# see--/speech_recognition

Measured on AMD Instinct MI355X. Metric: 1s 16kHz clips/sec training throughput, higher is better.
Workload: dtype f32; 1 GPU; configs[1]: 12-class conv_1d_time_sliced_with_attention, batch 1024/GPU synthetic 16000-sample fp32 clips, sampler+augment+STFT/mel(80,60)+raw fwd/bwd+RMSprop; global_batch=1024, parallelism=dp1, clip_bank=65536

## Files before the change

### include/kws_hip.h

```cpp
#ifndef KWS_HIP_H_
#define KWS_HIP_H_

#include <stdint.h>

#ifdef __cplusplus
extern "C" {
#endif
#if defined(__GNUC__) || defined(__clang__)
#pragma GCC visibility push(default)
#endif

#define KWS_OK 0
#define KWS_E_INVALID (-1)
#define KWS_E_HIP (-2)
#define KWS_E_WORKSPACE (-3)

#define KWS_ABI_VERSION 5

int kws_abi_version(void);
const char* kws_last_error(void);
int kws_device_name(char* buf, int cap);

int kws_stream_create(int cls, void** stream);
int kws_stream_destroy(void* stream);
// ... 186 lines not shown
                       void* stream);
int kws_conv1d_dgrad_f32(const float* dY, const float* W, float* dX, int accumulate, const kws_conv1d_t* d, void* stream);
int64_t kws_conv1d_wgrad_workspace_floats(const kws_conv1d_t* d);
int kws_conv1d_wgrad_f32(const float* X, const float* bn, const float* dY, float* dW, float* workspace, const kws_conv1d_t* d,
                         void* stream);

int kws_avgpool3_same_fwd_f32(const float* x, const float* bn, float* z, int B, int L, int C, void* stream);
int kws_avgpool3_same_bwd_f32(const float* dz, float* dx, int accumulate, int B, int L, int C, void* stream);

#define KWS_ACT_RELU6 0
#define KWS_ACT_RELU 1
typedef struct {
  int B, H, W, Hout, Wout;
  int kh, kw;
  int sh, sw;
  int dh, dw;
  int pad_t, pad_l;
  int Cin, F;
  int act;
} kws_conv2d_t;
int kws_conv2d_stats_rows(const kws_conv2d_t* d);
int kws_conv2d_fwd_f32(const float* X, const float* bn, const float* Wt, float* Y, float* stats_part, const kws_conv2d_t* d,
                       void* stream);
int kws_conv2d_dgrad_f32(const float* dY, const float* Wt, float* dX, const kws_conv2d_t* d, void* stream);
int64_t kws_conv2d_wgrad_workspace_floats(const kws_conv2d_t* d);
int kws_conv2d_wgrad_f32(const float* X, const float* bn, const float* dY, float* dWt, float* workspace, const kws_conv2d_t* d,
                         void* stream);

int kws_pool2x2_fwd_f32(const float* y, const float* bn, float* z, int B, int H, int W, int C, int act, void* stream);
int kws_pool2x2_bwd_part_rows(int B, int H, int W, int C);
int64_t kws_pool2x2_bwd_part_floats(int B, int H, int W, int C);
int kws_pool2x2_bwd_f32(const float* dz, const float* y, const float* bn, float* g, float* part, int B, int H, int W, int C, int act,
                        void* stream);

typedef struct {
  int B, L, Lout;
  int ksize, hop, pad_l;
  int taps, stride;
  int N;
  int64_t x_batch_stride;
} kws_frame_conv_t;
int kws_frame_conv_stats_rows(const kws_frame_conv_t* d);
int kws_frame_conv_fwd_f32(const float* x, const float* W, float* y, float* stats_part, const kws_frame_conv_t* d, void* stream);
int64_t kws_frame_conv_wgrad_workspace_floats(const kws_frame_conv_t* d);
int kws_frame_conv_wgrad_f32(const float* x, const float* G, float* dW, float* workspace, const kws_frame_conv_t* d, void* stream);

typedef struct {
  int B, L, Lout;
  int stride;
  int nbanks, N;
  int ksize[8], pad_l[8];
  int64_t w_off[8];
  int64_t x_batch_stride;
} kws_fbank_conv_t;
int     kws_fbank_conv_fwd_f32(const float* x, const float* W, float* y, const kws_fbank_conv_t* d, void* stream);
int64_t kws_fbank_conv_wgrad_workspace_floats(const kws_fbank_conv_t* d);
int     kws_fbank_conv_wgrad_f32(const float* x, const float* G, float* dW, float* workspace, const kws_fbank_conv_t* d, void* stream);

int kws_gap_drop_fwd_f32(const float* y, const float* bn, float* feat, float* fd, int B, int T, int C, float keep_prob, uint64_t seed,
                         uint32_t step, uint32_t layer_id, int64_t row_offset, void* stream);
int kws_gap_drop_bwd_part_rows(int B, int T, int C);
int kws_gap_drop_bwd_f32(const float* dfd, const float* y, const float* bn, float* g, float* part, int B, int T, int C, float keep_prob,
                         uint64_t seed, uint32_t step, uint32_t layer_id, int64_t row_offset, void* stream);

#define KWS_REDUCE_SLICES 32
int kws_bn_stats_finalize(const float* stats_part, int n_tiles, int64_t count, int C,
                          const float* gamma, const float* beta, float eps, float momentum,
                          float* moving_mean, float* moving_var, float* bn, float* scratch,
                          void* stream);
int kws_bn_infer_prepare(const float* gamma, const float* beta, const float* moving_mean,
                         const float* moving_var, float eps, int C, float* bn, void* stream);
int kws_bn_relu6_apply(const float* y, const float* bn, float* out, int64_t rows, int C, int relu6,
                       void* stream);

int kws_dwconv_fwd_f32(const float* y, const float* bn, const float* w, float* z, int B, int L_in,
                       int L_out, int C, int stride, int pad_l, void* stream);
int64_t kws_dwconv_bwd_part_floats(int B, int L_in, int C);
int kws_dwconv_bwd_f32(const float* dz, const float* y, const float* bn, const float* w, float* g,
                       float* part, int B, int L_in, int L_out, int C, int stride, int pad_l,
                       void* stream);
int kws_dwconv_bwd_bn_f32(const float* dz, const float* y, const float* bn, const float* w,
                          const float* coef, float* dy, float* part, int pass, int B, int L_in,
                          int L_out, int C, int stride, int pad_l, void* stream);
int kws_dw_bwd_finalize(const float* part, int n_parts, int64_t count, int C, float* dw,
                        float* dgamma, float* dbeta, float* coef, float* scratch, void* stream);
int kws_bn_bwd_apply(float* g, const float* y, const float* bn, const float* gamma,
                     const float* coef, int64_t rows, int C, void* stream);

int kws_dwconvk_fwd_f32(const float* y, const float* bn, const float* w, float* z, int B, int L_in, int L_out, int C,
                        int k, int stride, int pad_l, void* stream);
int kws_dwconvk_bwd_part_rows(int B, int L_in, int C, int k, int stride);
int64_t kws_dwconvk_bwd_part_floats(int B, int L_in, int C, int k, int stride);
int kws_dwconvk_bwd_f32(const float* dz, const float* y, const float* bn, const float* w, float* g, float* part, int B,
                        int L_in, int L_out, int C, int k, int stride, int pad_l, void* stream);
int kws_dwconvk_bwd_finalize(const float* part, int n_parts, int64_t count, int C, int k, float* dw, float* dgamma,
                             float* dbeta, float* coef, void* stream);
int kws_dwconvk_pw1_stats_rows(int64_t M);
int kws_dwconvk_pw1_fwd_f32(const float* z, const float* p, float* y, int64_t M, int N, float* stats_part, void* stream);
int64_t kws_dwconvk_pw1_bwd_workspace_floats(int64_t M, int N);
int kws_dwconvk_pw1_bwd_f32(const float* dy, const float* z, const float* p, float* dz, float* dp, int64_t M, int N,
                            float* workspace, void* stream);

int kws_stem_stats_rows(int B, int L);
int kws_stem_fwd_f32(const float* x, const float* w, const float* p, float* y, int B, int L, int C, int N, float* stats_part,
                     void* stream);
int64_t kws_stem_bwd_workspace_floats(int B, int L, int C, int N);
int kws_stem_bwd_f32(const float* dy, const float* x, const float* w, const float* p, float* dw, float* dp, int B, int L, int C,
                     int N, float* workspace, void* stream);

int64_t kws_gru_save_floats(int B, int T, int H);
int64_t kws_gru_workspace_floats(int B, int T, int I, int H, int backward);
int kws_gru_masks(float* mx, float* mh, int B, int I, int H, float keep_prob, uint64_t seed, uint32_t step, int64_t row_offset,
                  void* stream);
int kws_gru_seq_fwd_f32(const float* a, int64_t dir_stride, int64_t gate_stride, int row_stride, const float* U0, const float* U1,
                        const float* bias0, const float* bias1, const float* mh, float* out, float* save, int B, int T, int H,
                        void* stream);
int kws_gru_seq_bwd_f32(const float* dout, const float* UT, const float* mh, const float* save, float* da, float* lop, int B, int T,
                        int H, void* stream);
int kws_gru_fwd_f32(const float* x, const float* W0, const float* U0, const float* bias0, const float* W1, const float* U1,
                    const float* bias1, const float* mx, const float* mh, float* out, float* save, float* workspace, int B, int T,
                    int I, int H, void* stream);
int kws_gru_bwd_f32(const float* dout, const float* x, const float* W0, const float* U0, const float* W1, const float* U1,
                    const float* mx, const float* mh, const float* save, float* dx, float* dW0, float* dU0, float* dbias0, float* dW1,
                    float* dU1, float* dbias1, float* workspace, int B, int T, int I, int H, void* stream);

int64_t kws_attn_gate_fwd_floats(int B, int T, int C, int k);
int64_t kws_attn_gate_bwd_floats(int B, int T, int C, int k);
int kws_attn_gate_fwd_f32(const float* x, const float* wa, const float* Wa, const float* gamma, const float* beta, float* mm,
                          float* mv, float* u, float* table, float* att, float* y, float* workspace, int B, int T, int C, int k,
                          int training, void* stream);
int kws_attn_gate_bwd_f32(const float* dy, const float* x, const float* u, const float* att, const float* table, const float* wa,
                          const float* Wa, const float* gamma, float* dx, float* dwa, float* dWa, float* dgamma, float* dbeta,
                          float* workspace, int B, int T, int C, int k, int training, void* stream);

int kws_rmsprop_step(float* p, const float* grad, float* acc, const float* l2, int64_t n, float lr,
                     float rho, float eps, float grad_scale, void* stream);
int kws_sgd_momentum_step(float* p, const float* grad, float* vel, const float* l2, int64_t n,
                          float lr, float momentum, float grad_scale, void* stream);
int kws_adam_step(float* p, const float* grad, float* m, float* v, const float* l2, int64_t n, float lr_t,
                  float beta1, float beta2, float eps, float grad_scale, void* stream);
int kws_l2_loss(const float* p, const float* l2, int64_t n, float* out, void* stream);

#define KWS_NET_TS_ATTENTION 1
#define KWS_NET_LOG_MFCC 2
#define KWS_NET_STEFFE 3
#define KWS_NET_RESIDUAL 4
#define KWS_NET_MFCC_AND_RAW 5
#define KWS_NET_CONV_1D_FAST 6
#define KWS_NET_CONV_1D_SPEC 7
#define KWS_NET_CONV_1D_TIME_STACKED 8
#define KWS_NET_CONV_1D_HEAVY 9
#define KWS_NET_CONV_1D_GRU 10
#define KWS_NET_CONV_1D_MULTI_TIME_SLICED 11
#define KWS_NET_CONV_1D_SIMPLE 12
#define KWS_NET_XCEPTION_ATTENTION 13
#define KWS_NET_INCEPTION_D1 14
#define KWS_NET_CONV_2D_MOBILE 15
#define KWS_NET_CONV_2D_FAST 16
#define KWS_NET_CONV_1D_TIME_SLICED 17
#define KWS_NET_CONV_1D_LEARNED_SPEC 18
#define KWS_NET_CONV_1D_TOP_DOWN 19
typedef struct kws_net kws_net_t;
typedef struct {
  int kind;
  int num_classes;
  int filter_mult;
// ... 50 lines not shown
```

### speech_recognition_amd/_lib.py

```python
import ctypes
import os

_HERE = os.path.dirname(os.path.abspath(__file__))
LIB_PATH = os.environ.get("KWS_LIB_PATH") or os.path.join(_HERE, "libkws_hip.so")

ABI_VERSION = 5

KWS_NET_TS_ATTENTION = 1
KWS_NET_LOG_MFCC = 2
KWS_NET_STEFFE = 3
KWS_NET_RESIDUAL = 4
KWS_NET_MFCC_AND_RAW = 5
KWS_NET_CONV_1D_FAST = 6
KWS_NET_CONV_1D_SPEC = 7
KWS_NET_CONV_1D_TIME_STACKED = 8
KWS_NET_CONV_1D_HEAVY = 9
KWS_NET_CONV_1D_GRU = 10
KWS_NET_CONV_1D_MULTI_TIME_SLICED = 11
KWS_NET_CONV_1D_SIMPLE = 12
KWS_NET_XCEPTION_ATTENTION = 13
KWS_NET_INCEPTION_D1 = 14
KWS_NET_CONV_2D_MOBILE = 15
KWS_NET_CONV_2D_FAST = 16
KWS_NET_CONV_1D_TIME_SLICED = 17
# ... 145 lines not shown
    "kws_gemm_tn_f16x2_f32": (_I, [_P, _P, _P, _I64, _I, _I, _P, _P, _P, _P]),
    "kws_gemm_gather_f32": (_I, [_P, ctypes.POINTER(GatherDesc), _P, _P, _I, _I, _P, _P]),
    "kws_gemm_tn_workspace_floats": (_I64, [_I64, _I, _I]),
    "kws_gemm_tn_f32": (_I, [_P, _P, _P, _I64, _I, _I, _P, _P]),
    "kws_gemm_tn_gather_f32": (_I, [_P, ctypes.POINTER(GatherDesc), _P, _P, _I, _I, _P, _P]),
    "kws_gconv_stats_rows": (_I, [ctypes.POINTER(GconvDesc)]),
    "kws_gconv_fwd_f32": (_I, [_P, _P, _I, _P, _P, _P, ctypes.POINTER(GconvDesc), _P]),
    "kws_gconv_dgrad_f32": (_I, [_P, _P, _P, ctypes.POINTER(GconvDesc), _P]),
    "kws_gconv_wgrad_workspace_floats": (_I64, [ctypes.POINTER(GconvDesc)]),
    "kws_gconv_wgrad_f32": (_I, [_P, _P, _I, _P, _P, _P, ctypes.POINTER(GconvDesc), _P]),
    "kws_gdwconv_fwd_f32": (_I, [_P, _P, _P, _P, ctypes.POINTER(GdwconvDesc), _P]),
    "kws_gdwconv_bwd_part_rows": (_I, [ctypes.POINTER(GdwconvDesc)]),
    "kws_gdwconv_bwd_workspace_floats": (_I64, [ctypes.POINTER(GdwconvDesc)]),
    "kws_gdwconv_bwd_f32": (_I, [_P, _P, _P, _P, _P, _P, _P, _P, ctypes.POINTER(GdwconvDesc), _P]),
    "kws_pool3s2_out_len": (_I, [_I]),
    "kws_pool3s2_fwd_f32": (_I, [_P, _P, _P, _I, _I, _I, _P]),
    "kws_pool3s2_bwd_part_rows": (_I, [_I, _I, _I]),
    "kws_pool3s2_bwd_part_floats": (_I64, [_I, _I, _I]),
    "kws_pool3s2_bwd_f32": (_I, [_P, _P, _P, _P, _P, _I, _I, _I, _P]),
    "kws_pool3s2_same_out_len": (_I, [_I]),
    "kws_pool3s2_same_fwd_f32": (_I, [_P, _P, _P, _I, _I, _I, _P]),
    "kws_pool3s2_same_bwd_part_rows": (_I, [_I, _I, _I]),
    "kws_pool3s2_same_bwd_part_floats": (_I64, [_I, _I, _I]),
    "kws_pool3s2_same_bwd_f32": (_I, [_P, _P, _P, _P, _P, _I, _I, _I, _P]),
    "kws_conv1d_stats_rows": (_I, [ctypes.POINTER(Conv1dDesc)]),
    "kws_conv1d_fwd_f32": (_I, [_P, _P, _P, _P, _P, ctypes.POINTER(Conv1dDesc), _P]),
    "kws_conv1d_dgrad_f32": (_I, [_P, _P, _P, _I, ctypes.POINTER(Conv1dDesc), _P]),
    "kws_conv1d_wgrad_workspace_floats": (_I64, [ctypes.POINTER(Conv1dDesc)]),
    "kws_conv1d_wgrad_f32": (_I, [_P, _P, _P, _P, _P, ctypes.POINTER(Conv1dDesc), _P]),
    "kws_conv2d_stats_rows": (_I, [ctypes.POINTER(Conv2dDesc)]),
    "kws_conv2d_fwd_f32": (_I, [_P, _P, _P, _P, _P, ctypes.POINTER(Conv2dDesc), _P]),
    "kws_conv2d_dgrad_f32": (_I, [_P, _P, _P, ctypes.POINTER(Conv2dDesc), _P]),
    "kws_conv2d_wgrad_workspace_floats": (_I64, [ctypes.POINTER(Conv2dDesc)]),
    "kws_conv2d_wgrad_f32": (_I, [_P, _P, _P, _P, _P, ctypes.POINTER(Conv2dDesc), _P]),
    "kws_pool2x2_fwd_f32": (_I, [_P, _P, _P, _I, _I, _I, _I, _I, _P]),
    "kws_pool2x2_bwd_part_rows": (_I, [_I, _I, _I, _I]),
    "kws_pool2x2_bwd_part_floats": (_I64, [_I, _I, _I, _I]),
    "kws_pool2x2_bwd_f32": (_I, [_P, _P, _P, _P, _P, _I, _I, _I, _I, _I, _P]),
    "kws_frame_conv_stats_rows": (_I, [ctypes.POINTER(FrameConvDesc)]),
    "kws_frame_conv_fwd_f32": (_I, [_P, _P, _P, _P, ctypes.POINTER(FrameConvDesc), _P]),
    "kws_frame_conv_wgrad_workspace_floats": (_I64, [ctypes.POINTER(FrameConvDesc)]),
    "kws_frame_conv_wgrad_f32": (_I, [_P, _P, _P, _P, ctypes.POINTER(FrameConvDesc), _P]),
    "kws_fbank_conv_fwd_f32": (_I, [_P, _P, _P, ctypes.POINTER(FbankConvDesc), _P]),
    "kws_fbank_conv_wgrad_workspace_floats": (_I64, [ctypes.POINTER(FbankConvDesc)]),
    "kws_fbank_conv_wgrad_f32": (_I, [_P, _P, _P, _P, ctypes.POINTER(FbankConvDesc), _P]),
    "kws_gap_drop_fwd_f32": (_I, [_P, _P, _P, _P, _I, _I, _I, _F, ctypes.c_uint64, ctypes.c_uint32, ctypes.c_uint32, _I64, _P]),
    "kws_gap_drop_bwd_part_rows": (_I, [_I, _I, _I]),
    "kws_gap_drop_bwd_f32": (_I, [_P, _P, _P, _P, _P, _I, _I, _I, _F, ctypes.c_uint64, ctypes.c_uint32, ctypes.c_uint32, _I64,
                                  _P]),
    "kws_avgpool3_same_fwd_f32": (_I, [_P, _P, _P, _I, _I, _I, _P]),
    "kws_avgpool3_same_bwd_f32": (_I, [_P, _P, _I, _I, _I, _I, _P]),
    "kws_stem_stats_rows": (_I, [_I, _I]),
    "kws_stem_fwd_f32": (_I, [_P, _P, _P, _P, _I, _I, _I, _I, _P, _P]),
    "kws_stem_bwd_workspace_floats": (_I64, [_I, _I, _I, _I]),
    "kws_stem_bwd_f32": (_I, [_P, _P, _P, _P, _P, _P, _I, _I, _I, _I, _P, _P]),
    "kws_dwconvk_fwd_f32": (_I, [_P, _P, _P, _P, _I, _I, _I, _I, _I, _I, _I, _P]),
    "kws_dwconvk_bwd_part_rows": (_I, [_I, _I, _I, _I, _I]),
    "kws_dwconvk_bwd_part_floats": (_I64, [_I, _I, _I, _I, _I]),
    "kws_dwconvk_bwd_f32": (_I, [_P, _P, _P, _P, _P, _P, _I, _I, _I, _I, _I, _I, _I, _P]),
    "kws_dwconvk_bwd_finalize": (_I, [_P, _I, _I64, _I, _I, _P, _P, _P, _P, _P]),
    "kws_dwconvk_pw1_stats_rows": (_I, [_I64]),
    "kws_dwconvk_pw1_fwd_f32": (_I, [_P, _P, _P, _I64, _I, _P, _P]),
    "kws_dwconvk_pw1_bwd_workspace_floats": (_I64, [_I64, _I]),
    "kws_dwconvk_pw1_bwd_f32": (_I, [_P, _P, _P, _P, _P, _I64, _I, _P, _P]),
    "kws_gru_save_floats": (_I64, [_I, _I, _I]),
    "kws_gru_workspace_floats": (_I64, [_I, _I, _I, _I, _I]),
    "kws_gru_masks": (_I, [_P, _P, _I, _I, _I, _F, ctypes.c_uint64, ctypes.c_uint32, _I64, _P]),
    "kws_gru_seq_fwd_f32": (_I, [_P, _I64, _I64, _I, _P, _P, _P, _P, _P, _P, _P, _I, _I, _I, _P]),
    "kws_gru_seq_bwd_f32": (_I, [_P, _P, _P, _P, _P, _P, _I, _I, _I, _P]),
    "kws_gru_fwd_f32": (_I, [_P] * 12 + [_I, _I, _I, _I, _P]),
    "kws_gru_bwd_f32": (_I, [_P] * 17 + [_I, _I, _I, _I, _P]),
    "kws_attn_gate_fwd_floats": (_I64, [_I, _I, _I, _I]),
    "kws_attn_gate_bwd_floats": (_I64, [_I, _I, _I, _I]),
    "kws_attn_gate_fwd_f32": (_I, [_P] * 12 + [_I, _I, _I, _I, _I, _P]),
    "kws_attn_gate_bwd_f32": (_I, [_P] * 14 + [_I, _I, _I, _I, _I, _P]),
    "kws_transpose_f32": (_I, [_P, _P, _I, _I, _P]),
    "kws_bn_stats_finalize": (_I, [_P, _I, _I64, _I, _P, _P, _F, _F, _P, _P, _P, _P, _P]),
    "kws_bn_infer_prepare": (_I, [_P, _P, _P, _P, _F, _I, _P, _P]),
    "kws_bn_relu6_apply": (_I, [_P, _P, _P, _I64, _I, _I, _P]),
    "kws_dwconv_fwd_f32": (_I, [_P, _P, _P, _P, _I, _I, _I, _I, _I, _I, _P]),
    "kws_dwconv_bwd_part_floats": (_I64, [_I, _I, _I]),
    "kws_dwconv_bwd_f32": (_I, [_P, _P, _P, _P, _P, _P, _I, _I, _I, _I, _I, _I, _P]),
    "kws_dwconv_bwd_bn_f32": (_I, [_P, _P, _P, _P, _P, _P, _P, _I, _I, _I, _I, _I, _I, _I, _P]),
    "kws_dw_bwd_finalize": (_I, [_P, _I, _I64, _I, _P, _P, _P, _P, _P, _P]),
    "kws_bn_bwd_apply": (_I, [_P, _P, _P, _P, _P, _I64, _I, _P]),
    "kws_rmsprop_step": (_I, [_P, _P, _P, _P, _I64, _F, _F, _F, _F, _P]),
    "kws_sgd_momentum_step": (_I, [_P, _P, _P, _P, _I64, _F, _F, _F, _P]),
    "kws_adam_step": (_I, [_P, _P, _P, _P, _P, _I64, _F, _F, _F, _F, _F, _P]),
    "kws_l2_loss": (_I, [_P, _P, _I64, _P, _P]),
    "kws_net_create": (_I, [ctypes.POINTER(NetConfig), ctypes.POINTER(_P)]),
    "kws_net_destroy": (_I, [_P]),
    "kws_net_num_params": (_I64, [_P]),
    "kws_net_num_state": (_I64, [_P]),
    "kws_net_num_tensors": (_I, [_P]),
    "kws_net_tensor_info": (_I, [_P, _I, ctypes.POINTER(TensorInfo)]),
    "kws_net_workspace_bytes": (_I64, [_P, _I, _I]),
    "kws_net_debug_view": (_I, [_P, _I, _I, _I, _I, ctypes.POINTER(_I64), ctypes.POINTER(_I64)]),
    "kws_net_predict": (_I, [_P, _P, _P, _P, _I, _P, _P, _I64, _P]),
    "kws_net_train_fwd_bwd": (_I, [_P, _P, _P, _P, _P, _I, _P, _P, _P, ctypes.c_uint64, ctypes.c_uint32,
                                   _I64, _I, _P, _I64, _P]),
    "kws_net_num_blocks": (_I, [_P]),
    "kws_net_grad_ready_offset": (_I64, [_P, _I]),
    "kws_net_train_fwd_bwd_part": (_I, [_P, _P, _P, _P, _P, _I, _P, _P, _P, ctypes.c_uint64, ctypes.c_uint32,
                                        _I64, _I, _P, _I64, _I, _I, _P]),
}

_lib = None


def load():
    global _lib
    if _lib is not None:
        return _lib
    if not os.path.exists(LIB_PATH):
        raise KwsError("libkws_hip.so not found at %s - build it with "
                       "`python -c 'import __graft_entry__ as g; g.build()'` "
                       "(there is no CPU fallback)" % LIB_PATH)
    lib = ctypes.CDLL(LIB_PATH)
    lib.kws_abi_version.restype = _I
    if lib.kws_abi_version() != ABI_VERSION:
        raise KwsError("%s has ABI version %d, this package expects %d - rebuild it (__graft_entry__.build())" %
                       (LIB_PATH, lib.kws_abi_version(), ABI_VERSION))
    for name, (res, args) in SIGNATURES.items():
        fn = getattr(lib, name)
        fn.restype = res
        fn.argtypes = args
    _lib = lib
    return lib


def check(rc, what=""):
    if rc != 0:
        msg = load().kws_last_error()
        raise KwsError("%s failed (%d): %s" % (what or "libkws_hip call", rc,
                                               msg.decode() if msg else "?"))


def ptr(t):
    if t is None:
        return None
    return ctypes.c_void_p(t.data_ptr())


def stream_ptr(stream=None):
    import torch
    s = stream if stream is not None else torch.cuda.current_stream()
    return ctypes.c_void_p(s.cuda_stream)


class OwnedStream(object):

    def __init__(self, device, cls):
        import torch
        self.device = device
        with torch.cuda.device(device):
            h = ctypes.c_void_p()
            check(load().kws_stream_create(int(cls), ctypes.byref(h)), "kws_stream_create")
            self.handle = h.value
            self.stream = torch.cuda.ExternalStream(h.value, device=device)

    def close(self):
        h, self.handle = self.handle, None
        if h and _lib is not None:
            try:
                import torch
                with torch.cuda.device(self.device):
# ... 55 lines not shown
```

### speech_recognition_amd/csrc/dw_bwd_body.h

```cpp
#pragma once
#include "internal.h"

namespace kws_dw {

#ifndef KWS_DW_NT
#define KWS_DW_NT 1
#endif
typedef float dw_v4f __attribute__((ext_vector_type(4)));
__device__ __forceinline__ float4 ld4_stream(const float* p) {
  if (KWS_DW_NT & 2) {
    const dw_v4f v = __builtin_nontemporal_load(reinterpret_cast<const dw_v4f*>(p));
    return make_float4(v.x, v.y, v.z, v.w);
  }
  return *reinterpret_cast<const float4*>(p);
}
__device__ __forceinline__ void st4_stream(float* p, float4 o) {
  if (KWS_DW_NT & 1) {
    dw_v4f v = {o.x, o.y, o.z, o.w};
    __builtin_nontemporal_store(v, reinterpret_cast<dw_v4f*>(p));
    return;
  }
  *reinterpret_cast<float4*>(p) = o;
}

#ifndef KWS_DW_TT
#define KWS_DW_TT 8
#endif
constexpr int TT = KWS_DW_TT;

__device__ __forceinline__ float4 f4_fma(float4 a, float4 b, float4 c) {
  return make_float4(fmaf(a.x, b.x, c.x), fmaf(a.y, b.y, c.y), fmaf(a.z, b.z, c.z), fmaf(a.w, b.w, c.w));
}
__device__ __forceinline__ float4 f4_mul(float4 a, float4 b) {
  return make_float4(a.x * b.x, a.y * b.y, a.z * b.z, a.w * b.w);
}
__device__ __forceinline__ float4 f4_zero() { return make_float4(0.f, 0.f, 0.f, 0.f); }

#ifndef DW_BWD_THREADS
#define DW_BWD_THREADS 512
#endif
#ifndef DW_BWD_HT
#define DW_BWD_HT 8
#endif
#ifndef DW_BWD2_THREADS
#define DW_BWD2_THREADS 512
#endif
#ifndef DW_BWD_PARTS
#define DW_BWD_PARTS 256
#endif

struct BwdArgs {
  const float* dz; const float* y; const float* bn; const float* w; const float* coef;
  float* g; float* part;
  int B, Lin, Lout, C, pad_l, nchunks, R, Cb;
  unsigned* amax;
  int add_stride = 0, add_len = 0;
};
constexpr int bwd_smem_floats(int mode, int threads) { return mode == 2 ? 4 : 5 * threads * 4; }

template <int S, bool HAS_BN, int MODE, bool GUARD, bool ADDS = false>
__device__ __forceinline__ void bwd_body(const BwdArgs& p, float* const red, const int bid, const int nblk, const int by) {
  const float* __restrict__ dz = p.dz;
  const float* __restrict__ y = p.y;
  const float* __restrict__ bn = p.bn;
  const float* __restrict__ w = p.w;
  const float* __restrict__ coef = p.coef;
  float* __restrict__ g = p.g;
  float* __restrict__ part = p.part;
  const int B = p.B, Lin = p.Lin, Lout = p.Lout, C = p.C, pad_l = p.pad_l, nchunks = p.nchunks, R = p.R, Cb = p.Cb;
  constexpr int RSTRIDE = (MODE == 2 ? 4 : DW_BWD_THREADS * 4);
  float gmax = 0.f;
  const int C4 = Cb >> 2;
  const int tid = threadIdx.x;
  const bool live = !GUARD || tid < R * C4;
  const int r = live ? tid / C4 : 0, c4 = live ? tid - r * C4 : 0;
  const int c = by * Cb + c4 * 4;
  float4 sg = f4_zero(), sgx = f4_zero(), sw0 = f4_zero(), sw1 = f4_zero(), sw2 = f4_zero();
  float4 sc = f4_zero(), sh = f4_zero(), mean = f4_zero(), rstd = f4_zero();
  if (HAS_BN) {
    sc = *reinterpret_cast<const float4*>(bn + c);
    sh = *reinterpret_cast<const float4*>(bn + C + c);
    mean = *reinterpret_cast<const float4*>(bn + 2 * C + c);
    rstd = *reinterpret_cast<const float4*>(bn + 3 * C + c);
// ... 42 lines not shown
        if (u >= Lin) continue;
        float4 d0, d1, d2;
        if (S == 1) {
          d0 = D[i + 2]; d1 = D[i + 1]; d2 = D[i];
        } else if ((i & 1) == 0) {
          d0 = podd ? f4_zero() : D[i / 2 + 1];
          d2 = podd ? f4_zero() : D[i / 2];
          d1 = podd ? D[i / 2 + 1] : f4_zero();
        } else {
          d0 = podd ? D[(i + 1) / 2 + 1] : f4_zero();
          d2 = podd ? D[(i + 1) / 2] : f4_zero();
          d1 = podd ? f4_zero() : D[(i - 1) / 2 + 1];
        }
        const float4 yy = yv[i];
        float4 a = yy, mk = make_float4(1.f, 1.f, 1.f, 1.f), xh = f4_zero();
        if (HAS_BN) {
          const float4 pre = make_float4(fmaf(yy.x, sc.x, sh.x), fmaf(yy.y, sc.y, sh.y), fmaf(yy.z, sc.z, sh.z),
                                         fmaf(yy.w, sc.w, sh.w));
          a = make_float4(relu6f(pre.x), relu6f(pre.y), relu6f(pre.z), relu6f(pre.w));
          mk = make_float4((pre.x > 0.f && pre.x <= 6.f) ? 1.f : 0.f, (pre.y > 0.f && pre.y <= 6.f) ? 1.f : 0.f,
                           (pre.z > 0.f && pre.z <= 6.f) ? 1.f : 0.f, (pre.w > 0.f && pre.w <= 6.f) ? 1.f : 0.f);
          xh = make_float4((yy.x - mean.x) * rstd.x, (yy.y - mean.y) * rstd.y, (yy.z - mean.z) * rstd.z,
                           (yy.w - mean.w) * rstd.w);
        }
        float4 da = f4_mul(w0, d0);
        da = f4_fma(w1, d1, da);
        da = f4_fma(w2, d2, da);
        const float4 gv = f4_mul(da, mk);
        if (MODE == 2) {
          float4 o;
          o.x = sc.x * (gv.x - c1.x - (yy.x - mean.x) * rstd.x * c2.x);
          o.y = sc.y * (gv.y - c1.y - (yy.y - mean.y) * rstd.y * c2.y);
          o.z = sc.z * (gv.z - c1.z - (yy.z - mean.z) * rstd.z * c2.z);
          o.w = sc.w * (gv.w - c1.w - (yy.w - mean.w) * rstd.w * c2.w);
          st4_stream(gb + (int64_t)u * C, o);
          gmax = kws_abs4max(gmax, o);
          continue;
        }
        if (MODE == 0) {
          float4 o = gv;
          if (coef != nullptr) {
            if (!ADDS) {
              const float4 ad = *reinterpret_cast<const float4*>(coef + (b * (int64_t)Lin + u) * C + c);
              o = make_float4(o.x + ad.x, o.y + ad.y, o.z + ad.z, o.w + ad.w);
            } else {
              const int q = u / p.add_stride;
              const bool on = q * p.add_stride == u && q < p.add_len;
              const float4 ad = *reinterpret_cast<const float4*>(coef + (b * (int64_t)p.add_len + (on ? q : 0)) * C + c);
              o = make_float4(on ? o.x + ad.x : o.x, on ? o.y + ad.y : o.y, on ? o.z + ad.z : o.z, on ? o.w + ad.w : o.w);
            }
          }
          st4_stream(gb + (int64_t)u * C, o);
        }
        sg.x += gv.x; sg.y += gv.y; sg.z += gv.z; sg.w += gv.w;
        sgx = f4_fma(gv, xh, sgx);
        sw0 = f4_fma(d0, a, sw0);
        sw1 = f4_fma(d1, a, sw1);
        sw2 = f4_fma(d2, a, sw2);
      }
    }
  }
  if (MODE == 2) {
    if (p.amax && live) kws_absmax_commit(p.amax, gmax);
    return;
  }
  if constexpr (MODE != 2) {
  if (live) {
    *reinterpret_cast<float4*>(&red[0 * RSTRIDE + tid * 4]) = sg;
    *reinterpret_cast<float4*>(&red[1 * RSTRIDE + tid * 4]) = sgx;
    *reinterpret_cast<float4*>(&red[2 * RSTRIDE + tid * 4]) = sw0;
    *reinterpret_cast<float4*>(&red[3 * RSTRIDE + tid * 4]) = sw1;
    *reinterpret_cast<float4*>(&red[4 * RSTRIDE + tid * 4]) = sw2;
  }
  __syncthreads();
  for (int o = tid; o < 5 * Cb; o += blockDim.x) {
    const int q = o / Cb, ch = o - q * Cb;
    float s = 0.f;
    for (int rr = 0; rr < R; ++rr) s += red[q * RSTRIDE + (rr * C4) * 4 + ch];
    part[((int64_t)bid * 5 + q) * C + by * Cb + ch] = s;
  }
  }
}

constexpr int KWS_DW_BWD_MAX_PARTS = DW_BWD_PARTS;
struct BwdGeom {
  int nchunks, R, block, ny, Cb;
  int64_t grid;
};
inline bool bwd_geom_ok(int C) { return C > 0 && C % 4 == 0 && (C / 4) % ceil_div(C / 4, 256) == 0; }
inline BwdGeom bwd_geom(int B, int Lin, int C, bool parts = true) {
  BwdGeom g;
  const int threads = parts ? DW_BWD_THREADS : DW_BWD2_THREADS;
  const int max_parts = parts ? KWS_DW_BWD_MAX_PARTS : 1024;
  g.ny = ceil_div(C / 4, 256);
  g.Cb = C / g.ny;
  const int C4 = g.Cb / 4;
  g.nchunks = ceil_div(Lin, TT);
  g.R = threads / C4;
  if (g.R < 1) g.R = 1;
  g.block = g.R * C4;
  g.grid = ceil_div64((int64_t)B * g.nchunks, g.R);
  if (g.grid > max_parts) g.grid = max_parts;
  return g;
}

}
```

### speech_recognition_amd/csrc/dwconv.hip

```cpp
#include "dw_bwd_body.h"

namespace {
using namespace kws_dw;

#ifndef DW_FWD_GRID
#define DW_FWD_GRID 4096
#endif

template <int S, bool HAS_BN>
__global__ __launch_bounds__(256) void dwconv_fwd_kernel(const float* __restrict__ y, const float* __restrict__ bn,
                                                         const float* __restrict__ w, float* __restrict__ z,
                                                         int B, int Lin, int Lout, int C, int pad_l, int nchunks,
                                                         unsigned* amax) {
  const int C4 = C >> 2;
  float zmax = 0.f;
  const int64_t total = (int64_t)B * nchunks * C4;
  for (int64_t id = (int64_t)blockIdx.x * 256 + threadIdx.x; id < total; id += (int64_t)gridDim.x * 256) {
    const int c4 = (int)(id % C4);
    const int64_t rest = id / C4;
    const int chunk = (int)(rest % nchunks);
    const int64_t b = rest / nchunks;
    const int c = c4 * 4;
    float4 sc = f4_zero(), sh = f4_zero();
    if (HAS_BN) {
      sc = *reinterpret_cast<const float4*>(bn + c);
      sh = *reinterpret_cast<const float4*>(bn + C + c);
    }
    const float4 w0 = *reinterpret_cast<const float4*>(w + c);
    const float4 w1 = *reinterpret_cast<const float4*>(w + C + c);
    const float4 w2 = *reinterpret_cast<const float4*>(w + 2 * C + c);
    const float* yb = y + b * (int64_t)Lin * C + c;
    float* zb = z + b * (int64_t)Lout * C + c;
    constexpr int NL = S == 1 ? TT + 2 : 2 * TT + 1;
    const int t0 = chunk * TT;
    const int u_lo = S * t0 - pad_l;
    float4 av[NL];
#pragma unroll
    for (int k = 0; k < NL; ++k) {
      const int u = u_lo + k;
      av[k] = ld4_stream(yb + (int64_t)(u >= 0 && u < Lin ? u : 0) * C);
    }
#pragma unroll
    for (int k = 0; k < NL; ++k) {
      const int u = u_lo + k;
      float4 v = av[k];
      if (HAS_BN) {
        v.x = relu6f(fmaf(v.x, sc.x, sh.x));
        v.y = relu6f(fmaf(v.y, sc.y, sh.y));
        v.z = relu6f(fmaf(v.z, sc.z, sh.z));
        v.w = relu6f(fmaf(v.w, sc.w, sh.w));
      }
      av[k] = u >= 0 && u < Lin ? v : f4_zero();
    }
#pragma unroll
    for (int i = 0; i < TT; ++i) {
      const int t = t0 + i;
      if (t >= Lout) continue;
      float4 o = f4_mul(w0, av[S * i]);
      o = f4_fma(w1, av[S * i + 1], o);
      o = f4_fma(w2, av[S * i + 2], o);
      st4_stream(zb + (int64_t)t * C, o);
      zmax = kws_abs4max(zmax, o);
    }
  }
  if (amax) kws_absmax_commit(amax, zmax);
}

#ifndef KWS_DW_BWD2_MINW
#define KWS_DW_BWD2_MINW 1
#endif
#ifndef KWS_DW_BWD1_MINW
#define KWS_DW_BWD1_MINW 1
#endif
template <int S, bool HAS_BN, int MODE, bool ADDS = false>
__global__ __launch_bounds__(MODE == 2 ? DW_BWD2_THREADS : DW_BWD_THREADS, MODE == 2 ? KWS_DW_BWD2_MINW : KWS_DW_BWD1_MINW) void dwconv_bwd_kernel(BwdArgs p) {
  __shared__ float red[bwd_smem_floats(MODE, DW_BWD_THREADS)];
  bwd_body<S, HAS_BN, MODE, false, ADDS>(p, red, (int)blockIdx.x, (int)gridDim.x, (int)blockIdx.y);
}

}


namespace {
template <int MODE>
int launch_dw_bwd(const float* dz, const float* y, const float* bn, const float* w, const float* coef, float* g,
                  float* part, int B, int L_in, int L_out, int C, int stride, int pad_l, hipStream_t st,
                  unsigned* amax = nullptr, int add_stride = 0, int add_len = 0) {
  const BwdGeom ge = bwd_geom(B, L_in, C, MODE != 2);
  KWS_REQUIRE(ge.grid < 0x7FFFFFFF, "dwconv_bwd: grid too large");
  dim3 gr((unsigned)ge.grid, (unsigned)ge.ny), b((unsigned)ge.block);
  BwdArgs a;
  a.dz = dz; a.y = y; a.bn = bn; a.w = w; a.coef = coef; a.g = g; a.part = part;
  a.B = B; a.Lin = L_in; a.Lout = L_out; a.C = C; a.pad_l = pad_l; a.nchunks = ge.nchunks; a.R = ge.R; a.Cb = ge.Cb; a.amax = amax;
  a.add_stride = add_stride; a.add_len = add_len;
  if (MODE == 0 && add_stride > 1) {
    if (stride == 1) hipLaunchKernelGGL((dwconv_bwd_kernel<1, false, MODE, true>), gr, b, 0, st, a);
    else hipLaunchKernelGGL((dwconv_bwd_kernel<2, false, MODE, true>), gr, b, 0, st, a);
    KWS_LAUNCH_CHECK("dwconv_bwd_kernel");
    return KWS_OK;
  }
  if (stride == 1) {
    if (bn) hipLaunchKernelGGL((dwconv_bwd_kernel<1, true, MODE>), gr, b, 0, st, a);
    else hipLaunchKernelGGL((dwconv_bwd_kernel<1, false, MODE>), gr, b, 0, st, a);
  } else {
    if (bn) hipLaunchKernelGGL((dwconv_bwd_kernel<2, true, MODE>), gr, b, 0, st, a);
    else hipLaunchKernelGGL((dwconv_bwd_kernel<2, false, MODE>), gr, b, 0, st, a);
  }
  KWS_LAUNCH_CHECK("dwconv_bwd_kernel");
  return KWS_OK;
}
}

extern "C" {

int kws_dwconv_fwd_f32(const float* y, const float* bn, const float* w, float* z, int B, int L_in, int L_out,
                       int C, int stride, int pad_l, void* stream) {
  return kws_dwconv_fwd_amax_f32(y, bn, w, z, B, L_in, L_out, C, stride, pad_l, nullptr, (hipStream_t)stream);
}

int kws_dwconv_fwd_amax_f32(const float* y, const float* bn, const float* w, float* z, int B, int L_in, int L_out,
                            int C, int stride, int pad_l, unsigned* amax, void* stream_) {
  hipStream_t stream = (hipStream_t)stream_;
  KWS_REQUIRE(y && w && z, "dwconv_fwd: NULL pointer");
  KWS_REQUIRE(B > 0 && L_in > 0 && L_out > 0 && C > 0 && C % 4 == 0, "dwconv_fwd: bad shape B=%d L=%d->%d C=%d",
              B, L_in, L_out, C);
  KWS_REQUIRE(stride == 1 || stride == 2, "dwconv_fwd: stride %d unsupported", stride);
  KWS_REQUIRE(pad_l >= 0 && stride * (L_out - 1) + 2 - pad_l < L_in + 2, "dwconv_fwd: geometry reads past padding");
  const int nchunks = ceil_div(L_out, TT);
  const int64_t threads = (int64_t)B * nchunks * (C / 4);
  int64_t grid = ceil_div64(threads, 256);
  if (grid > DW_FWD_GRID) grid = DW_FWD_GRID;
  dim3 g((unsigned)grid), b(256);
  hipStream_t st = (hipStream_t)stream;
  KwsProfScope prof("dwconv_fwd", 6.0 * B * L_out * C, 4.0 * ((double)B * L_in * C + (double)B * L_out * C), st);
  if (stride == 1) {
    if (bn) hipLaunchKernelGGL((dwconv_fwd_kernel<1, true>), g, b, 0, st, y, bn, w, z, B, L_in, L_out, C, pad_l, nchunks, amax);
    else hipLaunchKernelGGL((dwconv_fwd_kernel<1, false>), g, b, 0, st, y, bn, w, z, B, L_in, L_out, C, pad_l, nchunks, amax);
  } else {
    if (bn) hipLaunchKernelGGL((dwconv_fwd_kernel<2, true>), g, b, 0, st, y, bn, w, z, B, L_in, L_out, C, pad_l, nchunks, amax);
    else hipLaunchKernelGGL((dwconv_fwd_kernel<2, false>), g, b, 0, st, y, bn, w, z, B, L_in, L_out, C, pad_l, nchunks, amax);
  }
  KWS_LAUNCH_CHECK("dwconv_fwd_kernel");
  return KWS_OK;
}

int64_t kws_dwconv_bwd_part_floats(int B, int L_in, int C) {
  if (B <= 0 || L_in <= 0 || !bwd_geom_ok(C)) return 0;
  const BwdGeom g = bwd_geom(B, L_in, C);
  return g.grid * 5 * C;
}

int kws_dwconv_bwd_f32(const float* dz, const float* y, const float* bn, const float* w, float* g, float* part,
                       int B, int L_in, int L_out, int C, int stride, int pad_l, void* stream) {
  KWS_REQUIRE(dz && y && w && g && part, "dwconv_bwd: NULL pointer");
  KWS_REQUIRE(B > 0 && L_in > 0 && L_out > 0 && bwd_geom_ok(C),
              "dwconv_bwd: bad shape B=%d L=%d->%d C=%d", B, L_in, L_out, C);
  KWS_REQUIRE(stride == 1 || stride == 2, "dwconv_bwd: stride %d unsupported", stride);
  hipStream_t st = (hipStream_t)stream;
  KwsProfScope prof("dwconv_bwd", 12.0 * B * L_in * C, 4.0 * (2.0 * B * L_in * C + (double)B * L_out * C), st);
  return launch_dw_bwd<0>(dz, y, bn, w, nullptr, g, part, B, L_in, L_out, C, stride, pad_l, st);
}

int kws_dwconv_bwd_acc_f32(const float* dz, const float* y, const float* w, const float* add, float* g, float* part, int B,
                           int L_in, int L_out, int C, int stride, int pad_l, hipStream_t st) {
  KWS_REQUIRE(dz && y && w && add && g && part && add != g, "dwconv_bwd_acc: bad pointers");
  KWS_REQUIRE(B > 0 && L_in > 0 && L_out > 0 && bwd_geom_ok(C) && (stride == 1 || stride == 2),
              "dwconv_bwd_acc: bad shape B=%d L=%d->%d C=%d stride=%d", B, L_in, L_out, C, stride);
  KwsProfScope prof("dwconv_bwd", 13.0 * B * L_in * C, 4.0 * (3.0 * B * L_in * C + (double)B * L_out * C), st);
  return launch_dw_bwd<0>(dz, y, nullptr, w, add, g, part, B, L_in, L_out, C, stride, pad_l, st);
}

int kws_dwconv_bwd_acc_strided_f32(const float* dz, const float* y, const float* w, const float* add, int add_stride, int add_len,
                                   float* g, float* part, int B, int L_in, int L_out, int C, int stride, int pad_l, hipStream_t st) {
  KWS_REQUIRE(dz && y && w && add && g && part && add != g, "dwconv_bwd_acc_strided: bad pointers");
  KWS_REQUIRE(B > 0 && L_in > 0 && L_out > 0 && bwd_geom_ok(C) && (stride == 1 || stride == 2) && add_stride >= 2 && add_len > 0 &&
                  (int64_t)(add_len - 1) * add_stride < L_in,
              "dwconv_bwd_acc_strided: bad shape B=%d L=%d->%d C=%d stride=%d add %d x %d", B, L_in, L_out, C, stride, add_len, add_stride);
  KwsProfScope prof("dwconv_bwd", 13.0 * B * L_in * C, 4.0 * (2.0 * B * L_in * C + (double)B * L_out * C + (double)B * add_len * C), st);
  return launch_dw_bwd<0>(dz, y, nullptr, w, add, g, part, B, L_in, L_out, C, stride, pad_l, st, nullptr, add_stride, add_len);
}

int kws_dwconv_bwd_bn_f32(const float* dz, const float* y, const float* bn, const float* w, const float* coef,
                          float* dy, float* part, int pass, int B, int L_in, int L_out, int C, int stride, int pad_l,
                          void* stream) {
  return kws_dwconv_bwd_bn_amax_f32(dz, y, bn, w, coef, dy, part, pass, B, L_in, L_out, C, stride, pad_l, nullptr,
                                    (hipStream_t)stream);
}

int kws_dwconv_bwd_bn_amax_f32(const float* dz, const float* y, const float* bn, const float* w, const float* coef,
                               float* dy, float* part, int pass, int B, int L_in, int L_out, int C, int stride, int pad_l,
                               unsigned* amax, void* stream_) {
  hipStream_t stream = (hipStream_t)stream_;
  KWS_REQUIRE(dz && y && bn && w, "dwconv_bwd_bn: NULL pointer");
  KWS_REQUIRE(pass == 1 ? part != nullptr : (pass == 2 && coef != nullptr && dy != nullptr),
              "dwconv_bwd_bn: pass %d needs %s", pass, pass == 1 ? "part" : "coef and dy");
  KWS_REQUIRE(B > 0 && L_in > 0 && L_out > 0 && bwd_geom_ok(C),
              "dwconv_bwd_bn: bad shape B=%d L=%d->%d C=%d", B, L_in, L_out, C);
  KWS_REQUIRE(stride == 1 || stride == 2, "dwconv_bwd_bn: stride %d unsupported", stride);
  hipStream_t st = (hipStream_t)stream;
  KwsProfScope prof("dwconv_bwd", 12.0 * B * L_in * C,
                    4.0 * ((pass == 2 ? 2.0 : 1.0) * B * L_in * C + (double)B * L_out * C), st);
  if (pass == 1) return launch_dw_bwd<1>(dz, y, bn, w, nullptr, nullptr, part, B, L_in, L_out, C, stride, pad_l, st);
  return launch_dw_bwd<2>(dz, y, bn, w, coef, dy, nullptr, B, L_in, L_out, C, stride, pad_l, st, amax);
}

}
```

Baseline: 227,000 clips/s.

## Wave-specialise depthwise conv backward pass 1 with async global-to-LDS loader waves

Adds a warp-specialised variant of the depthwise-conv backward BN pass-1 kernel. Extra loader waves stream y and dz tiles straight into an LDS ring buffer with global_load_lds, using vmcnt waits and barriers, while the compute waves accumulate the gradient and BN partial sums from LDS. The intent is to overlap memory latency with compute in this bandwidth-bound reduction. In exchange it uses a large LDS ring per block, which limits occupancy, and adds a bypass entry point that keeps the old register path available.

```diff
diff --git a/include/kws_hip.h b/include/kws_hip.h
--- a/include/kws_hip.h
+++ b/include/kws_hip.h
@@ -292,6 +292,8 @@
 int kws_dwconv_bwd_bn_f32(const float* dz, const float* y, const float* bn, const float* w,
                           const float* coef, float* dy, float* part, int pass, int B, int L_in,
                           int L_out, int C, int stride, int pad_l, void* stream);
+int kws_dwconv_bwd_bn_pass1_reg_f32(const float* dz, const float* y, const float* bn, const float* w, float* part, int B,
+                                    int L_in, int L_out, int C, int stride, int pad_l, void* stream);
 int kws_dw_bwd_finalize(const float* part, int n_parts, int64_t count, int C, float* dw,
                         float* dgamma, float* dbeta, float* coef, float* scratch, void* stream);
 int kws_bn_bwd_apply(float* g, const float* y, const float* bn, const float* gamma,
diff --git a/speech_recognition_amd/_lib.py b/speech_recognition_amd/_lib.py
--- a/speech_recognition_amd/_lib.py
+++ b/speech_recognition_amd/_lib.py
@@ -251,6 +251,7 @@
     "kws_dwconv_bwd_part_floats": (_I64, [_I, _I, _I]),
     "kws_dwconv_bwd_f32": (_I, [_P, _P, _P, _P, _P, _P, _I, _I, _I, _I, _I, _I, _P]),
     "kws_dwconv_bwd_bn_f32": (_I, [_P, _P, _P, _P, _P, _P, _P, _I, _I, _I, _I, _I, _I, _I, _P]),
+    "kws_dwconv_bwd_bn_pass1_reg_f32": (_I, [_P, _P, _P, _P, _P, _I, _I, _I, _I, _I, _I, _P]),
     "kws_dw_bwd_finalize": (_I, [_P, _I, _I64, _I, _P, _P, _P, _P, _P, _P]),
     "kws_bn_bwd_apply": (_I, [_P, _P, _P, _P, _P, _I64, _I, _P]),
     "kws_rmsprop_step": (_I, [_P, _P, _P, _P, _I64, _F, _F, _F, _F, _P]),
diff --git a/speech_recognition_amd/csrc/dw_bwd_body.h b/speech_recognition_amd/csrc/dw_bwd_body.h
--- a/speech_recognition_amd/csrc/dw_bwd_body.h
+++ b/speech_recognition_amd/csrc/dw_bwd_body.h
@@ -1,4 +1,5 @@
 #pragma once
+#include <type_traits>
 #include "internal.h"
 
 namespace kws_dw {
@@ -207,6 +208,232 @@
   }
 }
 
+#ifndef DW_WS_HS
+#define DW_WS_HS 2
+#endif
+#ifndef DW_WS_NT
+#define DW_WS_NT 0
+#endif
+static_assert(TT % DW_WS_HS == 0 && DW_WS_HS % 2 == 0, "DW_WS_HS must be even and divide TT");
+constexpr int WS_NST = TT / DW_WS_HS;
+constexpr int ws_nd_unit(int S) { return S == 1 ? TT + 2 : TT / 2 + 2; }
+constexpr int ws_dz_rows(int S, int k) { return (S == 1 ? DW_WS_HS : DW_WS_HS / 2) + (k == 0 ? 2 : 0); }
+constexpr int ws_dz_first(int S, int k) { return k == 0 ? 0 : ws_dz_rows(S, 0) + (k - 1) * ws_dz_rows(S, 1); }
+constexpr int ws_rows(int S, int k) { return DW_WS_HS + ws_dz_rows(S, k); }
+constexpr int ws_row0(int S, int k) { return k == 0 ? 0 : ws_rows(S, 0) + (k - 1) * ws_rows(S, 1); }
+constexpr int ws_total_rows(int S) { return TT + ws_nd_unit(S); }
+constexpr int ws_rows_after(int S, int k) { return ws_total_rows(S) - ws_row0(S, k) - ws_rows(S, k); }
+constexpr int ws_lds_f4(int S) { return ws_total_rows(S) * DW_BWD_THREADS; }
+static_assert(ws_row0(1, WS_NST - 1) + ws_rows(1, WS_NST - 1) == ws_total_rows(1) &&
+              ws_row0(2, WS_NST - 1) + ws_rows(2, WS_NST - 1) == ws_total_rows(2), "the slots tile the ring");
+static_assert(ws_lds_f4(1) * 16 <= 160 * 1024 && ws_lds_f4(2) * 4 >= bwd_smem_floats(1, DW_BWD_THREADS), "LDS ring size");
+
+typedef __attribute__((address_space(3))) void dw_lds_void;
+typedef const __attribute__((address_space(1))) void dw_glb_void;
+
+template <int K, int N, class F>
+__device__ __forceinline__ void ws_for(F&& f) {
+  if constexpr (K < N) {
+    f(std::integral_constant<int, K>{});
+    ws_for<K + 1, N>(f);
+  }
+}
+template <int N>
+__device__ __forceinline__ void ws_wait_vm() { asm volatile("s_waitcnt vmcnt(%0)" ::"n"(N) : "memory"); }
+
+struct WsCol { int y0, y_hi, d0, d_lo, d_hi; };
+
+template <int S, int NLW>
+__device__ __forceinline__ void ws_cols(const BwdArgs& p, const int lw, const int lane, const unsigned ub,
+                                        WsCol (&col)[DW_BWD_THREADS / 64 / NLW]) {
+  constexpr int CPW = DW_BWD_THREADS / 64 / NLW;
+  const int C = p.C, C4 = C >> 2, R = p.R, Lin = p.Lin, Lout = p.Lout;
+  const int block = R * C4, rowb = C * 4;
+#pragma unroll
+  for (int cc = 0; cc < CPW; ++cc) {
+    const int t = (lw + cc * NLW) * 64 + lane;
+    const bool live = t < block;
+    const int r = live ? t / C4 : 0, c4 = live ? t - r * C4 : 0;
+    const unsigned unit = ub * (unsigned)R + (unsigned)r;
+    unsigned b = unit / (unsigned)p.nchunks;
+    const int chunk = (int)(unit - b * (unsigned)p.nchunks);
+    if (b >= (unsigned)p.B) b = (unsigned)p.B - 1u;
+    const int u0 = chunk * TT;
+    const int y_lo = ((int)b * Lin * C4 + c4) * 16;
+    const int t_lo = S == 1 ? u0 + p.pad_l - 2 : ((u0 + p.pad_l) >> 1) - 1;
+    col[cc].y0 = y_lo + u0 * rowb;
+    col[cc].y_hi = y_lo + (Lin - 1) * rowb;
+    col[cc].d_lo = ((int)b * Lout * C4 + c4) * 16;
+    col[cc].d_hi = col[cc].d_lo + (Lout - 1) * rowb;
+    col[cc].d0 = col[cc].d_lo + t_lo * rowb;
+  }
+}
+
+template <int S, int NLW, int K>
+__device__ __forceinline__ void ws_offsets(const WsCol (&col)[DW_BWD_THREADS / 64 / NLW], const int rowb,
+                                           int (&off)[ws_rows(S, 0) * (DW_BWD_THREADS / 64 / NLW)]) {
+  constexpr int HS = DW_WS_HS, CPW = DW_BWD_THREADS / 64 / NLW, ROWS = ws_rows(S, K);
+#pragma unroll
+  for (int cc = 0; cc < CPW; ++cc) {
+#pragma unroll
+    for (int i = 0; i < HS; ++i) off[cc * ROWS + i] = min(col[cc].y0 + (K * HS + i) * rowb, col[cc].y_hi);
+#pragma unroll
+    for (int j = 0; j < ws_dz_rows(S, K); ++j)
+      off[cc * ROWS + HS + j] = min(max(col[cc].d0 + (ws_dz_first(S, K) + j) * rowb, col[cc].d_lo), col[cc].d_hi);
+  }
+}
+
+template <int S, int NLW, int K>
+__device__ __forceinline__ void ws_fire(const BwdArgs& p, float4* const ring, const int lw,
+                                        const int (&off)[ws_rows(S, 0) * (DW_BWD_THREADS / 64 / NLW)]) {
+  constexpr int HS = DW_WS_HS, CPW = DW_BWD_THREADS / 64 / NLW, ROWS = ws_rows(S, K);
+  const char* const yb = reinterpret_cast<const char*>(p.y);
+  const char* const dzb = reinterpret_cast<const char*>(p.dz);
+#pragma unroll
+  for (int cc = 0; cc < CPW; ++cc) {
+    float4* const dst = ring + ws_row0(S, K) * DW_BWD_THREADS + (lw + cc * NLW) * 64;
+#pragma unroll
+    for (int q = 0; q < ROWS; ++q)
+      __builtin_amdgcn_global_load_lds((dw_glb_void*)((q < HS ? yb : dzb) + (unsigned)off[cc * ROWS + q]),
+                                       (dw_lds_void*)(dst + q * DW_BWD_THREADS), 16, 0, DW_WS_NT ? 2 : 0);
+  }
+}
+
+template <int S, int NLW>
+__device__ __forceinline__ void bwd_ws_body(const BwdArgs& p, float4* const ring, const int bid, const int nblk) {
+  constexpr int HS = DW_WS_HS, NST = WS_NST, NDU = ws_nd_unit(S), CPW = DW_BWD_THREADS / 64 / NLW;
+  static_assert((DW_BWD_THREADS / 64) % NLW == 0 && (ws_total_rows(S) - ws_rows(S, 1)) * CPW <= 63,
+                "loader waves must divide the column groups; vmcnt holds 63");
+  const int B = p.B, Lin = p.Lin, Lout = p.Lout, C = p.C, pad_l = p.pad_l, nchunks = p.nchunks, R = p.R;
+  const int C4 = C >> 2;
+  const int tid = threadIdx.x;
+  const unsigned nunits = (unsigned)B * (unsigned)nchunks;
+  const unsigned nwu = (nunits + (unsigned)R - 1u) / (unsigned)R;
+  const int nit = (unsigned)bid < nwu ? (int)((nwu - 1u - (unsigned)bid) / (unsigned)nblk) + 1 : 0;
+  float4 sg = f4_zero(), sgx = f4_zero(), sw0 = f4_zero(), sw1 = f4_zero(), sw2 = f4_zero();
+  const bool live = tid < R * C4;
+  const int r = live ? tid / C4 : 0, c4 = live ? tid - r * C4 : 0;
+  const int c = c4 * 4;
+  const float4 sc = *reinterpret_cast<const float4*>(p.bn + c);
+  const float4 sh = *reinterpret_cast<const float4*>(p.bn + C + c);
+  const float4 mean = *reinterpret_cast<const float4*>(p.bn + 2 * C + c);
+  const float4 rstd = *reinterpret_cast<const float4*>(p.bn + 3 * C + c);
+  const float4 w0 = *reinterpret_cast<const float4*>(p.w + c);
+  const float4 w1 = *reinterpret_cast<const float4*>(p.w + C + c);
+  const float4 w2 = *reinterpret_cast<const float4*>(p.w + 2 * C + c);
+  asm volatile("" ::"v"(sc.x), "v"(sh.x), "v"(mean.x), "v"(rstd.x), "v"(w0.x), "v"(w1.x), "v"(w2.x));
+  if (tid >= DW_BWD_THREADS) {
+    const int lw = __builtin_amdgcn_readfirstlane((tid - DW_BWD_THREADS) >> 6), lane = tid & 63;
+    const int rowb = C * 4;
+    __builtin_amdgcn_s_setprio(3);
+    WsCol col[CPW];
+    int off[ws_rows(S, 0) * CPW];
+    if (nit > 0) {
+      ws_cols<S, NLW>(p, lw, lane, (unsigned)bid, col);
+      ws_for<0, NST>([&](auto kc) {
+        constexpr int K = decltype(kc)::value;
+        ws_offsets<S, NLW, K>(col, rowb, off);
+        ws_fire<S, NLW, K>(p, ring, lw, off);
+      });
+    }
+    for (int it = 0; it < nit; ++it) {
+      const bool more = it + 1 < nit;
+      if (more) ws_cols<S, NLW>(p, lw, lane, (unsigned)bid + (unsigned)(it + 1) * (unsigned)nblk, col);
+      ws_for<0, NST>([&](auto kc) {
+        constexpr int K = decltype(kc)::value;
+        if (more) ws_wait_vm<(ws_total_rows(S) - ws_rows(S, K)) * CPW>(); else ws_wait_vm<ws_rows_after(S, K) * CPW>();
+        __builtin_amdgcn_s_barrier();
+        asm volatile("" ::: "memory");
+        if (more) ws_offsets<S, NLW, K>(col, rowb, off);
+        __builtin_amdgcn_s_barrier();
+        asm volatile("" ::: "memory");
+        if (more) ws_fire<S, NLW, K>(p, ring, lw, off);
+      });
+    }
+  } else {
+    const bool podd = (pad_l & 1) != 0;
+    for (int it = 0; it < nit; ++it) {
+      const unsigned unit = ((unsigned)bid + (unsigned)it * (unsigned)nblk) * (unsigned)R + (unsigned)r;
+      const unsigned b = unit / (unsigned)nchunks;
+      const int chunk = (int)(unit - b * (unsigned)nchunks);
+      const int u0 = chunk * TT;
+      const bool act = live && b < (unsigned)B;
+      const int t_lo = S == 1 ? u0 + pad_l - 2 : ((u0 + pad_l) >> 1) - 1;
+      float4 D[NDU];
+      ws_for<0, NST>([&](auto kc) {
+        constexpr int K = decltype(kc)::value;
+        __syncthreads();
+        if (act && u0 + K * HS < Lin) {
+          const float4* const sb = ring + ws_row0(S, K) * DW_BWD_THREADS + tid;
+          float4 yv[HS];
+#pragma unroll
+          for (int i = 0; i < HS; ++i) yv[i] = sb[i * DW_BWD_THREADS];
+#pragma unroll
+          for (int j = 0; j < ws_dz_rows(S, K); ++j) D[ws_dz_first(S, K) + j] = sb[(HS + j) * DW_BWD_THREADS];
+#pragma unroll
+          for (int j = 0; j < ws_dz_rows(S, K); ++j) {
+            const int t = t_lo + ws_dz_first(S, K) + j;
+            if (t < 0 || t >= Lout) D[ws_dz_first(S, K) + j] = f4_zero();
+          }
+#pragma unroll
+          for (int ii = 0; ii < HS; ++ii) {
+            constexpr int i0 = K * HS;
+            const int i = i0 + ii;
+            const int u = u0 + i;
+            if (u >= Lin) continue;
+            float4 d0, d1, d2;
+            if (S == 1) {
+              d0 = D[i + 2]; d1 = D[i + 1]; d2 = D[i];
+            } else if ((i & 1) == 0) {
+              d0 = podd ? f4_zero() : D[i / 2 + 1];
+              d2 = podd ? f4_zero() : D[i / 2];
+              d1 = podd ? D[i / 2 + 1] : f4_zero();
+            } else {
+              d0 = podd ? D[(i + 1) / 2 + 1] : f4_zero();
+              d2 = podd ? D[(i + 1) / 2] : f4_zero();
+              d1 = podd ? f4_zero() : D[(i - 1) / 2 + 1];
+            }
+            const float4 yy = yv[ii];
+            const float4 pre = make_float4(fmaf(yy.x, sc.x, sh.x), fmaf(yy.y, sc.y, sh.y), fmaf(yy.z, sc.z, sh.z),
+                                           fmaf(yy.w, sc.w, sh.w));
+            const float4 a = make_float4(relu6f(pre.x), relu6f(pre.y), relu6f(pre.z), relu6f(pre.w));
+            const float4 mk = make_float4((pre.x > 0.f && pre.x <= 6.f) ? 1.f : 0.f, (pre.y > 0.f && pre.y <= 6.f) ? 1.f : 0.f,
+                                          (pre.z > 0.f && pre.z <= 6.f) ? 1.f : 0.f, (pre.w > 0.f && pre.w <= 6.f) ? 1.f : 0.f);
+            const float4 xh = make_float4((yy.x - mean.x) * rstd.x, (yy.y - mean.y) * rstd.y, (yy.z - mean.z) * rstd.z,
+                                          (yy.w - mean.w) * rstd.w);
+            float4 da = f4_mul(w0, d0);
+            da = f4_fma(w1, d1, da);
+            da = f4_fma(w2, d2, da);
+            const float4 gv = f4_mul(da, mk);
+            sg.x += gv.x; sg.y += gv.y; sg.z += gv.z; sg.w += gv.w;
+            sgx = f4_fma(gv, xh, sgx);
+            sw0 = f4_fma(d0, a, sw0);
+            sw1 = f4_fma(d1, a, sw1);
+            sw2 = f4_fma(d2, a, sw2);
+          }
+        }
+        __syncthreads();
+      });
+    }
+  }
+  constexpr int RSTRIDE = DW_BWD_THREADS * 4;
+  float* const red = reinterpret_cast<float*>(ring);
+  if (live && tid < DW_BWD_THREADS) {
+    *reinterpret_cast<float4*>(&red[0 * RSTRIDE + tid * 4]) = sg;
+    *reinterpret_cast<float4*>(&red[1 * RSTRIDE + tid * 4]) = sgx;
+    *reinterpret_cast<float4*>(&red[2 * RSTRIDE + tid * 4]) = sw0;
+    *reinterpret_cast<float4*>(&red[3 * RSTRIDE + tid * 4]) = sw1;
+    *reinterpret_cast<float4*>(&red[4 * RSTRIDE + tid * 4]) = sw2;
+  }
+  __syncthreads();
+  for (int o = tid; o < 5 * C; o += blockDim.x) {
+    const int q = o / C, ch = o - q * C;
+    float s = 0.f;
+    for (int rr = 0; rr < R; ++rr) s += red[q * RSTRIDE + (rr * C4) * 4 + ch];
+    p.part[((int64_t)bid * 5 + q) * C + ch] = s;
+  }
+}
+
 constexpr int KWS_DW_BWD_MAX_PARTS = DW_BWD_PARTS;
 struct BwdGeom {
   int nchunks, R, block, ny, Cb;
diff --git a/speech_recognition_amd/csrc/dwconv.hip b/speech_recognition_amd/csrc/dwconv.hip
--- a/speech_recognition_amd/csrc/dwconv.hip
+++ b/speech_recognition_amd/csrc/dwconv.hip
@@ -72,20 +72,39 @@
 #ifndef KWS_DW_BWD1_MINW
 #define KWS_DW_BWD1_MINW 1
 #endif
-template <int S, bool HAS_BN, int MODE, bool ADDS = false>
-__global__ __launch_bounds__(MODE == 2 ? DW_BWD2_THREADS : DW_BWD_THREADS, MODE == 2 ? KWS_DW_BWD2_MINW : KWS_DW_BWD1_MINW) void dwconv_bwd_kernel(BwdArgs p) {
-  __shared__ float red[bwd_smem_floats(MODE, DW_BWD_THREADS)];
-  bwd_body<S, HAS_BN, MODE, false, ADDS>(p, red, (int)blockIdx.x, (int)gridDim.x, (int)blockIdx.y);
+template <int S, bool HAS_BN, int MODE, bool ADDS = false, int WS = 0>
+__global__ __launch_bounds__((MODE == 2 ? DW_BWD2_THREADS : DW_BWD_THREADS) + 64 * WS, MODE == 2 ? KWS_DW_BWD2_MINW : KWS_DW_BWD1_MINW) void dwconv_bwd_kernel(BwdArgs p) {
+  if constexpr (WS > 0) {
+    static_assert(MODE == 1 && HAS_BN && !ADDS, "the wave-specialised form is pass 1 behind a BatchNorm");
+    __shared__ float4 ring[ws_lds_f4(S)];
+    bwd_ws_body<S, WS>(p, ring, (int)blockIdx.x, (int)gridDim.x);
+  } else {
+    __shared__ float red[bwd_smem_floats(MODE, DW_BWD_THREADS)];
+    bwd_body<S, HAS_BN, MODE, false, ADDS>(p, red, (int)blockIdx.x, (int)gridDim.x, (int)blockIdx.y);
+  }
 }
 
 }
 
 
 namespace {
+#ifndef DW_WS_LOADERS
+#define DW_WS_LOADERS 8
+#endif
+#ifndef DW_WS_MAX_C
+#define DW_WS_MAX_C 192
+#endif
+bool dw_ws_takes(const BwdGeom& ge, int B, int L_in, int C) {
+  if (ge.ny != 1 || ge.block > DW_BWD_THREADS || C > DW_WS_MAX_C) return false;
+  if ((int64_t)B * ge.nchunks + ge.R >= (int64_t)1 << 30) return false;
+  if (((int64_t)B * L_in + 4 * TT) * C * 4 >= (int64_t)1 << 31) return false;
+  return true;
+}
+
 template <int MODE>
 int launch_dw_bwd(const float* dz, const float* y, const float* bn, const float* w, const float* coef, float* g,
                   float* part, int B, int L_in, int L_out, int C, int stride, int pad_l, hipStream_t st,
-                  unsigned* amax = nullptr, int add_stride = 0, int add_len = 0) {
+                  unsigned* amax = nullptr, int add_stride = 0, int add_len = 0, bool reg_path = false) {
   const BwdGeom ge = bwd_geom(B, L_in, C, MODE != 2);
   KWS_REQUIRE(ge.grid < 0x7FFFFFFF, "dwconv_bwd: grid too large");
   dim3 gr((unsigned)ge.grid, (unsigned)ge.ny), b((unsigned)ge.block);
@@ -93,6 +112,15 @@
   a.dz = dz; a.y = y; a.bn = bn; a.w = w; a.coef = coef; a.g = g; a.part = part;
   a.B = B; a.Lin = L_in; a.Lout = L_out; a.C = C; a.pad_l = pad_l; a.nchunks = ge.nchunks; a.R = ge.R; a.Cb = ge.Cb; a.amax = amax;
   a.add_stride = add_stride; a.add_len = add_len;
+  if constexpr (MODE == 1) {
+    if (!reg_path && bn && dw_ws_takes(ge, B, L_in, C)) {
+      dim3 bw(DW_BWD_THREADS + 64 * DW_WS_LOADERS);
+      if (stride == 1) hipLaunchKernelGGL((dwconv_bwd_kernel<1, true, 1, false, DW_WS_LOADERS>), gr, bw, 0, st, a);
+      else hipLaunchKernelGGL((dwconv_bwd_kernel<2, true, 1, false, DW_WS_LOADERS>), gr, bw, 0, st, a);
+      KWS_LAUNCH_CHECK("dwconv_bwd_kernel");
+      return KWS_OK;
+    }
+  }
   if (MODE == 0 && add_stride > 1) {
     if (stride == 1) hipLaunchKernelGGL((dwconv_bwd_kernel<1, false, MODE, true>), gr, b, 0, st, a);
     else hipLaunchKernelGGL((dwconv_bwd_kernel<2, false, MODE, true>), gr, b, 0, st, a);
@@ -187,6 +215,14 @@
                                     (hipStream_t)stream);
 }
 
+int kws_dwconv_bwd_bn_pass1_reg_f32(const float* dz, const float* y, const float* bn, const float* w, float* part, int B, int L_in,
+                                    int L_out, int C, int stride, int pad_l, void* stream) {
+  KWS_REQUIRE(dz && y && bn && w && part, "dwconv_bwd_bn_pass1_reg: NULL pointer");
+  KWS_REQUIRE(B > 0 && L_in > 0 && L_out > 0 && bwd_geom_ok(C), "dwconv_bwd_bn_pass1_reg: bad shape B=%d L=%d->%d C=%d", B, L_in, L_out, C);
+  KWS_REQUIRE(stride == 1 || stride == 2, "dwconv_bwd_bn_pass1_reg: stride %d unsupported", stride);
+  return launch_dw_bwd<1>(dz, y, bn, w, nullptr, nullptr, part, B, L_in, L_out, C, stride, pad_l, (hipStream_t)stream, nullptr, 0, 0, true);
+}
+
 int kws_dwconv_bwd_bn_amax_f32(const float* dz, const float* y, const float* bn, const float* w, const float* coef,
                                float* dy, float* part, int pass, int B, int L_in, int L_out, int C, int stride, int pad_l,
                                unsigned* amax, void* stream_) {
```

Measured after the change: 227,100 clips/s, median of 2. No clear change (+0.0%).
